# Grice-Lab/HmmUFOtu

Hardware: AMD Instinct MI355X
Metric: reads placed/sec (whole node), gg_97_otus GTR+dGamma 250bp; HBM GB/s %peak (higher is better)
Workload: dtype f64; 1 GPU; gg_97_otus-scale synthetic DB (198643 nodes x 7682 CS columns, K=1400), GTR+dGamma(4), SE 250 bp amplicon reads, batch 8192 reads/step/GPU, 6 batches in flight, seeds in the reference's std::sort order (k_seed_refsort); seed_order=reference, message_window_cols=7682, parallelism=read-sharded x1

## Files before the change

hmmufotu_amd/csrc/hu_common.h:

```cpp
#pragma once
#include <hip/hip_runtime.h>
#include <stdint.h>
#include <string>
#include <functional>
#include <istream>
#include <ostream>
#include <vector>
#include <exception>
#include <mutex>
#include <thread>
#include "../../include/hmmufotu_amd.h"

#define HU_MAX_DGK 16
#define HU_READ_TILE 16
#define HU_MAX_INS 24
#define HU_TILEQ_MASK_SHIFT 16
#define HU_TILEW_QUAD (4 * HU_READ_TILE * 3)
#define HU_NODE_PAD 256
#define HU_MIN_LOGLIK_EXP (-510.0)
#define HU_BRANCH_EPS 1e-5
#define HU_MAX_ITER 100

struct HuModelDev {
	int32_t type, dgK;
	double pi[4];
	double logpi[4];
	double U[16], U1[16], lam[4];
	double rate[HU_MAX_DGK];
};

struct HuDbDev {
	int32_t nNodes, nNodesPad, csLen, W, WQ, root;
	int64_t winStart, winLen;
	const uint4* planes;
	const int32_t* posCol;
	const unsigned long long* colPlanes;
	int32_t QM, pad0;
	const uint2* nodeCover;
	const int32_t* parent;
	const double* blen;
	const double* height;
	const double* up;
	const double* down;
	const int32_t* upK;
	const int32_t* downK;
	int32_t K, L;
	const double* EM;
	const double* EI;
	const double* T;
	const double* entryC;
	const double* exitC;
	const int32_t* p2cs;
	const double* Tt;
	const double* EMt;
	const double* EIt;
	const double* placeConst;
	int32_t rLo, rHi;
	const uint32_t* wideList;
};
__device__ inline bool hu_skip_width(const HuDbDev& db, int cols) { return db.rHi != 0 && (cols <= db.rLo || cols > db.rHi); }

struct HuRegion {
	int32_t j0, j1, i0, i1;
	int32_t withB;
	int32_t band;
	int32_t from, start, nIns, nDel;
	int64_t off;
	int64_t doff;
	int32_t ci0, cj0;
	int64_t coff;
};
#define HU_MAX_REGIONS 6
#define HU_READ_NEEDS_VALUES 8

struct HuReadDesc {
	int64_t baseOff;
	int32_t len;
	int32_t nRegions;
	int64_t scratchOff;
	int64_t traceOff;
	int64_t decOff;
	int64_t cornerOff;
	HuRegion reg[HU_MAX_REGIONS];
};

void hu_set_error(const char* fmt, ...);
int hu_catch_all(const char* fn) noexcept;
void hu_sort_prefix_packed(uint64_t* a, size_t n, size_t k);

#define HU_PC_LAM 0
#define HU_PC_RATE 4
#define HU_PC_W 20
#define HU_PC_C 100
#define HU_PC_CB 164
#define HU_PC_S 184
#define HU_PC_COUNT 188
void hu_place_consts(const HuModelDev& m, double* pc);

int hu_model_prepare(const hu_model_desc* d, HuModelDev* out);

// ... 49 lines not shown
```

hmmufotu_amd/csrc/hu_engine.hip:

```cpp
#include <algorithm>
#include <cmath>
#include <cstdio>
#include <cstring>
#include <limits>
#include <map>
#include <atomic>
#include <thread>
#include <memory>
#include <mutex>
#include <chrono>
#include <fstream>
#include <sstream>
#include <new>
#include <stdexcept>
#include <fcntl.h>
#include <unistd.h>
#include "hu_common.h"
#include "hu_kern_sep.h"
#include "hu_kern_align.h"
#include "hu_kern_tree.h"
#include "hu_kern_blk.h"
#include "hu_kern_refsort.h"
#include "hu_kern_rank.h"
#include "hu_kern_anneal.h"
// ... 1841 lines not shown
			if(g2.i1 >= g2.i0 && g2.j1 >= g2.j0) { nearI = std::min(nearI, g2.i0 - 1); nearJ = std::min(nearJ, g2.j0 - 1); }
		}
		g.ci0 = std::max(g.i0, nearI); g.cj0 = std::max(g.j0, nearJ); g.coff = coff;
		if(nearI == INT32_MAX || g.ci0 > g.i1 || g.cj0 > g.j1 || g.i1 < g.i0 || g.j1 < g.j0) { g.ci0 = g.i1 + 1; g.cj0 = g.j1 + 1; }
		else coff += (int64_t)(g.i1 - g.ci0 + 1) * (g.j1 - g.cj0 + 1);
	}
	rd.scratchOff = off;
	rd.decOff = doff;
	rd.cornerOff = coff;
}

static int upload_descs(hu_batch* b) {
	int rc;
	if((rc = b->dDescs.ensure(b->hDescs.size())) != HU_OK) return rc;
	HIPCHK(hipMemcpyAsync(b->dDescs.p, b->hDescs.data(), b->hDescs.size() * sizeof(HuReadDesc), hipMemcpyHostToDevice, b->stream));
	return HU_OK;
}

extern "C" int hu_batch_set_reads(hu_batch* b, int n, const char* bases, const int64_t* offs, const int32_t* vpaths,
		const char* mates, const int64_t* moffs, const int32_t* mvpaths) try {
	if(!b || n < 0 || n > b->maxReads || (n > 0 && (!bases || !offs))) { hu_set_error("hu_batch_set_reads: bad argument"); return HU_ERR_ARG; }
	if(mates && !moffs) { hu_set_error("hu_batch_set_reads: mates without offsets"); return HU_ERR_ARG; }
	HIPCHK(hipSetDevice(b->db->device));
	b->n = n; b->paired = mates != nullptr; b->nSeq = b->paired ? 2 * n : n; b->fromCodes = false;
	b->hDescs.assign(b->nSeq, HuReadDesc());
	b->hBases.clear();
	b->maxBases = 0;
	for(int r = 0; r < n; ++r) {
		const int64_t l = (offs[r + 1] - offs[r]) + (mates ? moffs[r + 1] - moffs[r] : 0);
		if(l > b->maxBases) b->maxBases = (int) std::min<int64_t>(l, 1 << 30);
	}
	int64_t cells = 0, tr = 0, decs = 0, corners = 0;
	for(int s = 0; s < b->nSeq; ++s) {
		const bool isMate = s >= n;
		const int r = isMate ? s - n : s;
		const char* src = isMate ? mates + moffs[r] : bases + offs[r];
		const int64_t len64 = isMate ? moffs[r + 1] - moffs[r] : offs[r + 1] - offs[r];
		HuReadDesc& rd = b->hDescs[s];
		memset(&rd, 0, sizeof(rd));
		rd.baseOff = (int64_t) b->hBases.size();
		rd.len = (int32_t) len64;
		bool bad = len64 < 1 || len64 > 65535;
		for(int64_t i = 0; i < len64 && !bad; ++i) if(host_sym(src[i]) < 0) bad = true;
		if(!bad) {
			b->hBases.insert(b->hBases.end(), src, src + len64);
			const int32_t* vp = isMate ? (mvpaths ? mvpaths + (size_t) r * 12 : nullptr) : (vpaths ? vpaths + (size_t) r * 12 : nullptr);
			build_regions(b->db, rd.len, vp, rd);
			const int64_t c = rd.scratchOff, dc = rd.decOff, cc = rd.cornerOff;
			rd.scratchOff = cells; cells += c;
			rd.decOff = decs; decs += dc;
			rd.cornerOff = corners; corners += cc;
		}
		else { rd.len = 0; rd.nRegions = 0; }
		rd.traceOff = tr;
		tr += rd.len + b->db->dev.K + 8;
	}
	int rc;
	if((rc = b->dBases.ensure(b->hBases.size() + 1)) != HU_OK) return rc;
	b->cellsTotal = cells; b->cornerTotal = corners;
	if((rc = b->dDec.ensure((size_t) decs + 1)) != HU_OK) return rc;
	if((rc = b->dTraces.ensure((size_t) tr + 1)) != HU_OK) return rc;
	if((rc = b->dVit.ensure(b->nSeq)) != HU_OK) return rc;
	if(!b->hBases.empty()) HIPCHK(hipMemcpyAsync(b->dBases.p, b->hBases.data(), b->hBases.size(), hipMemcpyHostToDevice, b->stream));
	if((rc = upload_descs(b)) != HU_OK) return rc;
	b->state = ST_READS;
	return HU_OK;
} catch(...) { return hu_catch_all("hu_batch_set_reads"); }

static int ensure_read_buffers(hu_batch* b) {
	const HuDbDev& d = b->db->dev;
	const size_t n = (size_t) b->n;
	const size_t tiles = (n + HU_READ_TILE - 1) / HU_READ_TILE;
	int rc;
	if((rc = b->dCodes.ensure(n * d.csLen)) != HU_OK) return rc;
	if((rc = b->dStart.ensure(n)) != HU_OK) return rc;
	if((rc = b->dEnd.ensure(n)) != HU_OK) return rc;
	if((rc = b->dRp.ensure(tiles * d.WQ * HU_READ_TILE * 16)) != HU_OK) return rc;
	if((rc = b->dTileQ.ensure(tiles * (d.WQ + 1))) != HU_OK) return rc;
	if((rc = b->dTileW.ensure(std::max<size_t>(tiles, 1) * d.WQ * HU_TILEW_QUAD)) != HU_OK) return rc;
	if((rc = b->dSlotRead.ensure(std::max<size_t>(tiles, 1) * HU_READ_TILE)) != HU_OK) return rc;
	if((rc = b->dReadSlot.ensure(std::max<size_t>(n, 1))) != HU_OK) return rc;
	if((rc = b->dRq.ensure(std::max<size_t>(n, 1) * ((d.WQ + 31) / 32))) != HU_OK) return rc;
	if((rc = b->dIns.ensure(std::max<size_t>(n, 1) * (HU_MAX_INS + 1))) != HU_OK) return rc;
	if((rc = b->dTileIns.ensure(std::max<size_t>(tiles, 1) * (HU_READ_TILE * HU_MAX_INS + 1))) != HU_OK) return rc;
	if((rc = b->dRSpan.ensure(std::max<size_t>(n, 1) * 2)) != HU_OK) return rc;
	if((rc = b->dTileSpan.ensure(std::max<size_t>(tiles, 1) * 2)) != HU_OK) return rc;
	return HU_OK;
}

static int order_by_key(hu_batch* b, const uint32_t* key, const uint32_t* val, size_t n, uint32_t bound, uint32_t* out, bool runsInOrder) {
	if(!n) return HU_OK;
	const size_t m = (size_t) bound + 1;
	int rc;
	const size_t nTiles = (m + 1023) / 1024;
	if((rc = b->dCsCnt.ensure(3 * m + nTiles + 8)) != HU_OK) return rc;
	uint32_t* cnt = b->dCsCnt.p; uint32_t* start = cnt + m; uint32_t* cur = start + m + 1; uint32_t* tiles = cur + m;
	HIPCHK(hipMemsetAsync(cnt, 0, m * 4, b->stream));
	k_cs_hist<<<(unsigned)((n + 255) / 256), 256, 0, b->stream>>>((int) n, key, bound, cnt);
	k_cs_tile_sums<<<(unsigned) nTiles, 1024, 0, b->stream>>>((int) m, cnt, tiles);
	k_cs_scan_tiles<<<1, 1024, 0, b->stream>>>((int) nTiles, tiles);
	k_cs_scan<<<(unsigned) nTiles, 1024, 0, b->stream>>>((int) m, cnt, tiles, start, cur);
	k_cs_scatter<<<(unsigned)((n + 255) / 256), 256, 0, b->stream>>>((int) n, key, val, bound, cur, out);
	if(runsInOrder) k_cs_runs<<<(unsigned)((m + 3) / 4), 256, 0, b->stream>>>((int) bound, start, out);
	HIPCHK(hipGetLastError());
	return HU_OK;
}

static int tile_reads(hu_batch* b, const HuAlnDev* alns) {
	const int n = b->n;
	if(!n) return HU_OK;
	const int tiles = (n + HU_READ_TILE - 1) / HU_READ_TILE;
	int rc;
	if((rc = b->dSortK.ensure((size_t) n * 2)) != HU_OK || (rc = b->dSortV.ensure((size_t) n * 2)) != HU_OK) return rc;
	k_tile_keys<<<(n + 255) / 256, 256, 0, b->stream>>>(n, alns, b->dStart.p, b->dEnd.p, b->dSortK.p, b->dSortV.p);
	if(b->knob.tile_unsorted) HIPCHK(hipMemcpyAsync(b->dSortV.p + n, b->dSortV.p, (size_t) n * 4, hipMemcpyDeviceToDevice, b->stream));
	else if((rc = order_by_key(b, b->dSortK.p, b->dSortV.p, (size_t) n, (uint32_t) b->db->dev.csLen + 1u, b->dSortV.p + n, true)) != HU_OK) return rc;
	k_tile_slots<<<(tiles * HU_READ_TILE + 255) / 256, 256, 0, b->stream>>>(n, tiles * HU_READ_TILE, b->dSortV.p + n, b->dSlotRead.p, b->dReadSlot.p);
	HIPCHK(hipGetLastError());
	return HU_OK;
}

static int set_aligned_impl(hu_batch* b, int n, const int8_t* codes, hipMemcpyKind kind, const int32_t* start, const int32_t* end, int maxBases = -1) {
	if(!b || n < 0 || n > b->maxReads || (n > 0 && (!codes || !start || !end))) { hu_set_error("hu_batch_set_aligned: bad argument"); return HU_ERR_ARG; }
	HIPCHK(hipSetDevice(b->db->device));
	const HuDbDev& d = b->db->dev;
	b->n = n; b->nSeq = n; b->paired = false; b->fromCodes = true;
	if(maxBases >= 0) b->maxBases = maxBases;
	else {
		int mb = 0;
		for(int r = 0; r < n; ++r) {
			if(!(start[r] >= 0 && start[r] <= end[r] && end[r] < d.csLen)) continue;
			const int8_t* c = codes + (size_t) r * d.csLen; int k = 0;
			for(int j = start[r]; j <= end[r]; ++j) k += c[j] >= 0;
			mb = std::max(mb, k);
		}
		b->maxBases = mb;
	}
	int rc;
	if((rc = ensure_read_buffers(b)) != HU_OK) return rc;
	b->hAlns.assign(n, HuAlnDev());
	b->hStart.assign(start, start + n); b->hEnd.assign(end, end + n);
	for(int r = 0; r < n; ++r) {
		HuAlnDev& a = b->hAlns[r];
		memset(&a, 0, sizeof(a));
		const bool ok = start[r] >= 0 && start[r] <= end[r] && end[r] < d.csLen && start[r] >= d.winStart && end[r] < d.winStart + d.winLen;
		a.status = ok ? HU_READ_OK : HU_READ_INVALID;
		a.csStart = start[r] + 1; a.csEnd = end[r] + 1;
		if(!ok) { b->hStart[r] = (int32_t) d.winStart; b->hEnd[r] = (int32_t) d.winStart - 1; }
	}
	(void) hipGetLastError();
	if(n) {
		if((const void*) codes != (const void*) b->dCodes.p) HIPCHK(hipMemcpyAsync(b->dCodes.p, codes, (size_t) n * d.csLen, kind, b->stream));
		HIPCHK(hipMemcpyAsync(b->dStart.p, b->hStart.data(), (size_t) n * 4, hipMemcpyHostToDevice, b->stream));
		HIPCHK(hipMemcpyAsync(b->dEnd.p, b->hEnd.data(), (size_t) n * 4, hipMemcpyHostToDevice, b->stream));
		const int tiles = (n + HU_READ_TILE - 1) / HU_READ_TILE;
		HIPCHK(hipMemsetAsync(b->dRp.p, 0, (size_t) tiles * d.WQ * HU_READ_TILE * 16 * 4, b->stream));
		if((rc = tile_reads(b, nullptr)) != HU_OK) return rc;
		k_planes_from_codes<<<n, 64, 0, b->stream>>>(d, b->dCodes.p, b->dStart.p, b->dEnd.p, b->dRp.p, b->dRq.p, b->dIns.p, b->dReadSlot.p, (uint2*) b->dRSpan.p);
		k_tile_lists<<<tiles, 64, 0, b->stream>>>(d, n, b->dRp.p, b->dRq.p, b->dIns.p, b->dTileQ.p, b->dTileW.p, b->dTileIns.p, b->dSlotRead.p, (const uint2*) b->dRSpan.p, (uint2*) b->dTileSpan.p);
		HIPCHK(hipGetLastError());
	}
	b->state = ST_ALIGNED;
	return HU_OK;
}
extern "C" int hu_batch_set_aligned(hu_batch* b, int n, const int8_t* codes, const int32_t* start, const int32_t* end) try {
	return set_aligned_impl(b, n, codes, hipMemcpyHostToDevice, start, end);
} catch(...) { return hu_catch_all("hu_batch_set_aligned"); }
// ... 1975 lines not shown
```

hmmufotu_amd/csrc/hu_kern_align.h:

```cpp
#pragma once
#include "hu_common.h"

struct HuVitOut { int32_t alnStart, alnEnd, alnFrom, alnTo, traceLen, status; double minScore; };

__device__ inline bool reg_contains(const HuRegion& g, int i, int j) {
	if(j < g.j0 || j > g.j1 || i < g.i0 || i > g.i1) return false;
	if(g.band) { int dist = (i - g.from) - (j - g.start); if(!(dist <= g.nIns && dist >= -g.nDel)) return false; }
	return true;
}

struct VitCtx {
	const HuReadDesc* rd;
	const double* scr;
	double tNN, tNB;
};

__device__ inline void vit_lookup(const VitCtx& c, int upto, int i, int j, double& m, double& ii, double& d) {
	const HuReadDesc& rd = *c.rd;
	for(int r = upto - 1; r >= 0; --r) {
		const HuRegion& g = rd.reg[r];
		if(reg_contains(g, i, j)) {
			const int64_t idx = (g.off + (int64_t)(j - g.j0) * (g.i1 - g.i0 + 1) + (i - g.i0)) * 3;
			m = c.scr[idx]; ii = c.scr[idx + 1]; d = c.scr[idx + 2];
			return;
// ... 1060 lines not shown
	}
	if(lane == 0) {
		if(db.WQ & 31) qbits[(db.WQ - 1) >> 5] = acc; il[0] = li;
		rspan[r] = make_uint2((any1 ? f1 : 0xffffu) | ((any1 ? l1 : 0u) << 16), (any2 ? f2 : 0xffffu) | ((any2 ? l2 : 0u) << 16));
	}
}

__global__ __launch_bounds__(64) void k_encode_rows(HuDbDev db, const char* __restrict__ rows, HuAlnDev* __restrict__ alns,
		int8_t* __restrict__ codes, int32_t* __restrict__ rstart, int32_t* __restrict__ rend, uint32_t* __restrict__ rp, uint32_t* __restrict__ rq,
		int32_t* __restrict__ ins, const int32_t* __restrict__ readSlot, uint2* __restrict__ rspan) {
	const int r = blockIdx.x, lane = threadIdx.x;
	const HuAlnDev a = alns[r];
	const char* row = rows + (size_t) r * db.csLen;
	int8_t* cd = codes + (size_t) r * db.csLen;
	bool ok = a.status == HU_READ_OK;
	if(ok && (a.csStart - 1 < db.winStart || a.csEnd - 1 >= db.winStart + db.winLen)) {
		ok = false;
		if(lane == 0) alns[r].status = HU_READ_OUT_OF_WINDOW;
	}
	const int start = ok ? a.csStart - 1 : (int) db.winStart, end = ok ? a.csEnd - 1 : (int) db.winStart - 1;
	if(lane == 0) { rstart[r] = start; rend[r] = end; }
	for(int c = lane; c < db.csLen; c += 64) {
		char ch = row[c];
		if(ch >= 'a' && ch <= 'z') ch = (char)(ch - 32);
		cd[c] = c_sym_map[(int) ch & 127];
	}
	__syncthreads();
	planes_of_codes(db, cd, start, end, r, readSlot[r], lane, rp, rq, ins, rspan);
}

__global__ __launch_bounds__(64) void k_planes_from_codes(HuDbDev db, const int8_t* __restrict__ codes,
		const int32_t* __restrict__ rstart, const int32_t* __restrict__ rend, uint32_t* __restrict__ rp, uint32_t* __restrict__ rq,
		int32_t* __restrict__ ins, const int32_t* __restrict__ readSlot, uint2* __restrict__ rspan) {
	const int r = blockIdx.x, lane = threadIdx.x;
	planes_of_codes(db, codes + (size_t) r * db.csLen, rstart[r], rend[r], r, readSlot[r], lane, rp, rq, ins, rspan);
}

__global__ void k_tile_keys(int n, const HuAlnDev* __restrict__ alns, const int32_t* __restrict__ rstart, const int32_t* __restrict__ rend,
		uint32_t* __restrict__ key, uint32_t* __restrict__ val) {
	const int r = blockIdx.x * 256 + threadIdx.x;
	if(r >= n) return;
	uint32_t k;
	if(alns) k = alns[r].status == HU_READ_OK ? (uint32_t) alns[r].csStart : 0x7fffffffu;
	else k = rend[r] >= rstart[r] ? (uint32_t) rstart[r] + 1u : 0x7fffffffu;
	key[r] = k; val[r] = (uint32_t) r;
}
__global__ void k_tile_slots(int n, int nSlots, const uint32_t* __restrict__ sortedRead, int32_t* __restrict__ slotRead, int32_t* __restrict__ readSlot) {
	const int s = blockIdx.x * 256 + threadIdx.x;
	if(s >= nSlots) return;
	if(s < n) { const int r = (int) sortedRead[s]; slotRead[s] = r; readSlot[r] = s; }
	else slotRead[s] = -1;
}

__global__ __launch_bounds__(64) void k_tile_lists(HuDbDev db, int n, const uint32_t* __restrict__ rp, const uint32_t* __restrict__ rq, const int32_t* __restrict__ ins,
		int32_t* __restrict__ tileQ, uint32_t* __restrict__ tileW, int32_t* __restrict__ tileIns, const int32_t* __restrict__ slotRead, const uint2* __restrict__ rspan,
		uint2* __restrict__ tileSpan) {
	static_assert(HU_READ_TILE == 16, "sixteen reads x four validity words of a quad = one dword per lane");
	const int tile = blockIdx.x, lane = threadIdx.x;
	const int nw32 = (db.WQ + 31) / 32;
	int32_t* out = tileQ + (size_t) tile * (db.WQ + 1);
	uint32_t* wout = tileW + (size_t) tile * db.WQ * HU_TILEW_QUAD;
	int cnt = 0;
	for(int w = 0; w < nw32; ++w) {
		uint32_t m = 0;
		if(lane < HU_READ_TILE) { const int r = slotRead[tile * HU_READ_TILE + lane]; if(r >= 0) m = rq[(size_t) r * nw32 + w]; }
		for(int s = 32; s > 0; s >>= 1) m |= __shfl_xor(m, s);
		while(m) {
			const int q = w * 32 + __ffs(m) - 1; m &= m - 1;
			const uint32_t* __restrict__ rt = rp + ((size_t) tile * db.WQ + q) * (HU_READ_TILE * 16);
			unsigned long long b = __ballot(rt[(lane >> 2) * 16 + 8 + (lane & 3)] != 0u);
			b |= b >> 32; b |= b >> 16; b |= b >> 8; b |= b >> 4;
			uint32_t mk = (uint32_t) b & 15u;
			if(lane == 0) out[1 + cnt] = q | (int) mk << HU_TILEQ_MASK_SHIFT;
			++cnt;
			while(mk) {
				const int wd = __ffs(mk) - 1; mk &= mk - 1;
				if(lane < HU_READ_TILE * 3) wout[lane] = rt[(lane / 3) * 16 + (lane % 3) * 4 + wd];
				wout += HU_READ_TILE * 3;
			}
		}
	}
	if(lane == 0) {
		out[0] = cnt;
		int32_t* til = tileIns + (size_t) tile * (HU_READ_TILE * HU_MAX_INS + 1);
		int ne = 0;
		for(int t = 0; t < HU_READ_TILE; ++t) {
			const int r = slotRead[tile * HU_READ_TILE + t];
			if(r < 0) continue;
			const int32_t* il = ins + (size_t) r * (HU_MAX_INS + 1);
			for(int e = 0; e < il[0]; ++e) til[1 + ne++] = (t << 24) | il[1 + e];
		}
		til[0] = ne;
		uint32_t f1 = 0xffffu, l1 = 0, f2 = 0xffffu, l2 = 0; bool a1 = false, a2 = false;
		for(int t = 0; t < HU_READ_TILE; ++t) {
			const int r = slotRead[tile * HU_READ_TILE + t];
			if(r < 0) continue;
			const uint2 s2 = rspan[r];
			if((s2.x & 0xffffu) <= (s2.x >> 16)) { f1 = a1 ? min(f1, s2.x & 0xffffu) : (s2.x & 0xffffu); l1 = a1 ? max(l1, s2.x >> 16) : (s2.x >> 16); a1 = true; }
			if((s2.y & 0xffffu) <= (s2.y >> 16)) { f2 = a2 ? min(f2, s2.y & 0xffffu) : (s2.y & 0xffffu); l2 = a2 ? max(l2, s2.y >> 16) : (s2.y >> 16); a2 = true; }
		}
		tileSpan[tile] = make_uint2((a1 ? f1 : 0xffffu) | ((a1 ? l1 : 0u) << 16), (a2 ? f2 : 0xffffu) | ((a2 ? l2 : 0u) << 16));
	}
}
```

hmmufotu_amd/csrc/hu_kern_sep.h:

```cpp
#pragma once
#include "hu_common.h"

#define HU_TOPK_BINS 4097
#define HU_TOPK_CAP 4096

template<class PT> struct HuPair;
template<> struct HuPair<uint32_t> {
	static constexpr int PPV = 4;
	__device__ static inline uint32_t canon(uint32_t x) { return x; }
	__device__ static inline uint32_t pack(uint32_t c) { return c; }
	__device__ static inline void unpack(const uint4& v, uint32_t* o) { o[0] = v.x; o[1] = v.y; o[2] = v.z; o[3] = v.w; }
};
template<> struct HuPair<uint16_t> {
	static constexpr int PPV = 8;
	__device__ static inline uint32_t canon(uint32_t x) { return ((x >> 8) << 16) | (x & 0xffu); }
	__device__ static inline uint16_t pack(uint32_t c) { return (uint16_t)(((c >> 16) << 8) | (c & 0xffu)); }
	__device__ static inline void unpack(const uint4& v, uint32_t* o) {
		const uint32_t w[4] = {v.x, v.y, v.z, v.w};
#pragma unroll
		for(int e = 0; e < 8; ++e) o[e] = canon((w[e >> 1] >> ((e & 1) * 16)) & 0xffffu);
	}
};
__device__ inline uint32_t hu_pair_load(const void* pairs, size_t idx, int p16) {
	return p16 ? HuPair<uint16_t>::canon(((const uint16_t*) pairs)[idx]) : ((const uint32_t*) pairs)[idx];
}

__global__ __launch_bounds__(64) void k_col_planes(HuDbDev db, unsigned long long* __restrict__ col) {
	const int nb = blockIdx.x, q = db.QM + blockIdx.y, lane = threadIdx.x;
	const size_t np = (size_t) db.nNodesPad, npw = np / 64;
	const int node = nb * 64 + lane;
	for(int p = 0; p < 3; ++p) {
		const uint4 v = db.planes[((size_t) q * 3 + p) * np + node];
		const uint32_t w[4] = {v.x, v.y, v.z, v.w};
		for(int i = 0; i < 128; ++i) {
			const unsigned long long m = __ballot((w[i >> 5] >> (i & 31)) & 1u);
			if(lane == 0) col[(((size_t) blockIdx.y * 128 + i) * 3 + p) * npw + nb] = m;
		}
	}
}

__global__ __launch_bounds__(256) void k_node_cover(HuDbDev db, uint2* __restrict__ cover) {
	const int node = blockIdx.x * 256 + threadIdx.x;
	if(node >= db.nNodesPad) return;
	uint32_t f1 = 0xffffu, l1 = 0, f2 = 0xffffu, l2 = 0; bool any1 = false, any2 = false;
	for(int q = 0; q < db.WQ; ++q) {
		const uint4 v = db.planes[((size_t) q * 3 + 2) * db.nNodesPad + node];
		const uint32_t w[4] = {v.x, v.y, v.z, v.w};
		for(int k = 0; k < 4; ++k) {
			if(!w[k]) continue;
			const uint32_t lo = (uint32_t) q * 128 + k * 32 + (__ffs(w[k]) - 1), hi = (uint32_t) q * 128 + k * 32 + 31 - __clz(w[k]);
			if(q < db.QM) { if(!any1) { f1 = lo; any1 = true; } l1 = hi; }
			else { if(!any2) { f2 = lo; any2 = true; } l2 = hi; }
		}
	}
	cover[node] = make_uint2((any1 ? f1 : 0xffffu) | ((any1 ? l1 : 0u) << 16), (any2 ? f2 : 0xffffu) | ((any2 ? l2 : 0u) << 16));
}
__device__ inline bool hu_span_meets(uint32_t a, uint32_t b) {
	return (a & 0xffffu) <= (b >> 16) && (b & 0xffffu) <= (a >> 16) && (a & 0xffffu) <= (a >> 16) && (b & 0xffffu) <= (b >> 16);
}
__device__ inline bool hu_cover_meets(uint2 node, uint2 read) { return hu_span_meets(node.x, read.x) || hu_span_meets(node.y, read.y); }

template<int CTRL>
__device__ inline uint32_t dpp_min_full(uint32_t v) {
	const uint32_t o = (uint32_t) __builtin_amdgcn_mov_dpp((int) v, CTRL, 0xf, 0xf, true);
	return o < v ? o : v;
}
__device__ __forceinline__ void hu_scan_word(uint32_t n0, uint32_t n1, uint32_t nv, const uint32_t* __restrict__ r, uint32_t (&d)[HU_READ_TILE], uint32_t (&N)[HU_READ_TILE]) {
#pragma unroll
	for(int t = 0; t < HU_READ_TILE; ++t) {
		const uint32_t k = nv & r[t * 3 + 2], x = ((n0 ^ r[t * 3]) | (n1 ^ r[t * 3 + 1])) & k;
		d[t] += __popc(x); N[t] += __popc(k);
	}
}

template<class PT, bool L0 = false>
__global__ __launch_bounds__(256, 8) void k_seed_pdist2(HuDbDev db, const uint32_t* __restrict__ tileW,
		const int32_t* __restrict__ tileQ, const int32_t* __restrict__ tileIns, PT* __restrict__ pairs, const int32_t* __restrict__ slotRead,
		uint32_t* __restrict__ piv = nullptr, unsigned long long* __restrict__ l0m = nullptr) {
	constexpr int T = HU_READ_TILE;
	__shared__ uint32_t acc[T][256];
	const int tile = blockIdx.x, tid = threadIdx.x;
	const int node = blockIdx.y * 256 + tid;
	const int32_t* __restrict__ ql = tileQ + (size_t) tile * (db.WQ + 1);
	const int32_t* __restrict__ til = tileIns + (size_t) tile * (T * HU_MAX_INS + 1);
	const int nq = ql[0], ne = til[0];
	uint32_t d[T], N[T];
#pragma unroll
	for(int t = 0; t < T; ++t) { d[t] = 0; N[t] = 0; }
	if(ne) {
#pragma unroll
		for(int t = 0; t < T; ++t) acc[t][tid] = 0;
	}
	const size_t np = (size_t) db.nNodesPad;
	const uint32_t* __restrict__ wr = (const uint32_t*) __builtin_assume_aligned(tileW + (size_t) tile * db.WQ * HU_TILEW_QUAD, 64);
	for(int qi = 0; qi < nq; ++qi) {
		const int ent = ql[1 + qi], q = ent & ((1 << HU_TILEQ_MASK_SHIFT) - 1);
		const uint4 n0 = db.planes[((size_t) q * 3 + 0) * np + node], n1 = db.planes[((size_t) q * 3 + 1) * np + node], nv = db.planes[((size_t) q * 3 + 2) * np + node];
		if(ent & (1 << HU_TILEQ_MASK_SHIFT)) { hu_scan_word(n0.x, n1.x, nv.x, wr, d, N); wr += T * 3; }
		if(ent & (2 << HU_TILEQ_MASK_SHIFT)) { hu_scan_word(n0.y, n1.y, nv.y, wr, d, N); wr += T * 3; }
		if(ent & (4 << HU_TILEQ_MASK_SHIFT)) { hu_scan_word(n0.z, n1.z, nv.z, wr, d, N); wr += T * 3; }
		if(ent & (8 << HU_TILEQ_MASK_SHIFT)) { hu_scan_word(n0.w, n1.w, nv.w, wr, d, N); wr += T * 3; }
	}
	{
		const size_t npw = np / 64;
		const int nb = __builtin_amdgcn_readfirstlane(node >> 6), lane = tid & 63;
		for(int e = 0; e < ne; ++e) {
			const int ent = til[1 + e];
			const int t = ent >> 24, pos = (ent >> 2) & 0x3fffff, code = ent & 3;
			const unsigned long long* cp = db.colPlanes + ((size_t)(pos - db.QM * 128) * 3) * npw + nb;
			const unsigned long long W0 = cp[0], W1 = cp[npw], Wv = cp[2 * npw];
			const uint32_t valid = (uint32_t)(Wv >> lane) & 1u, nc = ((uint32_t)(W0 >> lane) & 1u) | (((uint32_t)(W1 >> lane) & 1u) << 1);
			const uint32_t add = valid | ((valid & (nc != (uint32_t) code ? 1u : 0u)) << 16);
			atomicAdd(&acc[t][tid], add);
		}
	}
	const bool counts = L0 && node < db.nNodes && node != db.root;
	bool zero = false;
#pragma unroll
	for(int t = 0; t < T; ++t) {
		const int read = slotRead[tile * T + t];
		if(read >= 0) {
			const uint32_t v = ((d[t] << 16) | N[t]) + (ne ? acc[t][tid] : 0u);
			pairs[(size_t) read * np + node] = HuPair<PT>::pack(v);
			if(L0) {
				const uint32_t pp = piv[(size_t) read * 4];
				const uint32_t a = (v >> 16) * (pp & 0xffffu), bb = (pp >> 16) * (v & 0xffffu);
				const unsigned long long mL = __ballot(counts && a >= bb), mR = __ballot(counts && bb >= a);
				if((tid & 63) == 0) *reinterpret_cast<ulonglong2*>(l0m + ((size_t) read * (np / 64) + (size_t)(node >> 6)) * 2) = make_ulonglong2(mL, mR);
				zero |= v == 0u;
			}
		}
	}
	if(L0 && __ballot(zero && counts)) {
#pragma unroll
		for(int t = 0; t < T; ++t) {
			const int read = slotRead[tile * T + t];
			if(read < 0) continue;
			const uint32_t v = ((d[t] << 16) | N[t]) + (ne ? acc[t][tid] : 0u);
			if(__ballot(counts && v == 0u) && (tid & 63) == 0) atomicOr(&piv[(size_t) read * 4 + 3], 1u);
		}
	}
}

template<class DT>
__global__ __launch_bounds__(256, 3) void k_seed_dscan4(HuDbDev db, const uint32_t* __restrict__ rp,
		const int32_t* __restrict__ tileQ, DT* __restrict__ dm, const int32_t* __restrict__ slotRead, uint32_t* __restrict__ bminD, const uint2* __restrict__ tileSpan) {
	constexpr int T = HU_READ_TILE, M = 4;
	constexpr uint32_t DMAX = (uint32_t)(DT) ~(DT) 0;
	static_assert(T == 16, "sixteen reads x sixteen dwords per quad = one dword per thread");
	__shared__ __attribute__((aligned(16))) uint32_t rpl2[2][T * 16];
	__shared__ __attribute__((aligned(16))) uint32_t mb[4][T][64];
	const int tile = blockIdx.x, tid = threadIdx.x, lane = tid & 63, wave = tid >> 6;
	const int node0 = blockIdx.y * (256 * M) + tid * M;
	const bool live = node0 < db.nNodesPad;
	const int nl = live ? node0 : 0;
	const int32_t* __restrict__ ql = tileQ + (size_t) tile * (db.WQ + 1);
	const int nq = ql[0];
	uint32_t d[T][M];
#pragma unroll
	for(int t = 0; t < T; ++t)
#pragma unroll
		for(int m = 0; m < M; ++m) d[t][m] = 0;
	const size_t np = (size_t) db.nNodesPad;
	for(int qi = 0; qi < nq; ++qi) {
		const int q = ql[1 + qi] & ((1 << HU_TILEQ_MASK_SHIFT) - 1);
		const uint32_t mine = rp[((size_t) tile * db.WQ + q) * (T * 16) + tid];
		uint4 n0[M], n1[M], nv[M];
#pragma unroll
		for(int m = 0; m < M; ++m) {
			n0[m] = db.planes[((size_t) q * 3 + 0) * np + nl + m]; n1[m] = db.planes[((size_t) q * 3 + 1) * np + nl + m]; nv[m] = db.planes[((size_t) q * 3 + 2) * np + nl + m];
		}
		uint32_t* rpl = rpl2[qi & 1];
		rpl[tid] = mine;
		__syncthreads();
		uint4 r0 = *reinterpret_cast<const uint4*>(&rpl[0]), r1 = *reinterpret_cast<const uint4*>(&rpl[4]), rv = *reinterpret_cast<const uint4*>(&rpl[8]);
#pragma unroll
		for(int t = 0; t < T; ++t) {
			const int tn = t + 1 < T ? t + 1 : t;
			const uint4 p0 = *reinterpret_cast<const uint4*>(&rpl[tn * 16]), p1 = *reinterpret_cast<const uint4*>(&rpl[tn * 16 + 4]), pv = *reinterpret_cast<const uint4*>(&rpl[tn * 16 + 8]);
			uint32_t a[M][4];
#pragma unroll
			for(int m = 0; m < M; ++m) { a[m][0] = n0[m].x ^ r0.x; a[m][1] = n0[m].y ^ r0.y; a[m][2] = n0[m].z ^ r0.z; a[m][3] = n0[m].w ^ r0.w; }
			__builtin_amdgcn_sched_barrier(0);
#pragma unroll
			for(int m = 0; m < M; ++m) {
				a[m][0] = __builtin_amdgcn_bitop3_b32(a[m][0], n1[m].x, r1.x, 0xf6); a[m][1] = __builtin_amdgcn_bitop3_b32(a[m][1], n1[m].y, r1.y, 0xf6);
				a[m][2] = __builtin_amdgcn_bitop3_b32(a[m][2], n1[m].z, r1.z, 0xf6); a[m][3] = __builtin_amdgcn_bitop3_b32(a[m][3], n1[m].w, r1.w, 0xf6);
			}
			__builtin_amdgcn_sched_barrier(0);
#pragma unroll
			for(int m = 0; m < M; ++m) {
				a[m][0] = __builtin_amdgcn_bitop3_b32(a[m][0], nv[m].x, rv.x, 0x80); a[m][1] = __builtin_amdgcn_bitop3_b32(a[m][1], nv[m].y, rv.y, 0x80);
				a[m][2] = __builtin_amdgcn_bitop3_b32(a[m][2], nv[m].z, rv.z, 0x80); a[m][3] = __builtin_amdgcn_bitop3_b32(a[m][3], nv[m].w, rv.w, 0x80);
			}
			__builtin_amdgcn_sched_barrier(0);
#pragma unroll
			for(int w = 0; w < 4; ++w) {
#pragma unroll
				for(int m = 0; m < M; ++m) asm("v_bcnt_u32_b32 %0, %1, %0" : "+v"(d[t][m]) : "v"(a[m][w]));
			}
			__builtin_amdgcn_sched_barrier(0);
			r0 = p0; r1 = p1; rv = pv;
		}
	}
	uint32_t skip[M];
	const uint2 tsp = tileSpan[tile];
#pragma unroll
	for(int m = 0; m < M; ++m) skip[m] = live && node0 + m < db.nNodes && node0 + m != db.root && hu_cover_meets(db.nodeCover[nl + m], tsp) ? 0u : 0xffffffffu;
#pragma unroll
	for(int t = 0; t < T; ++t) {
		const int read = slotRead[tile * T + t];
		uint32_t v[M];
#pragma unroll
		for(int m = 0; m < M; ++m) v[m] = min(d[t][m], DMAX);
		if(read >= 0 && live) {
			DT* dst = dm + (size_t) read * np + node0;
			if(sizeof(DT) == 1) *reinterpret_cast<uint32_t*>(dst) = v[0] | (v[1] << 8) | (v[2] << 16) | (v[3] << 24);
			else *reinterpret_cast<uint2*>(dst) = make_uint2(v[0] | (v[1] << 16), v[2] | (v[3] << 16));
		}
		mb[wave][t][lane] = min(min(v[0] | skip[0], v[1] | skip[1]), min(v[2] | skip[2], v[3] | skip[3]));
	}
	__syncthreads();
// ... 1224 lines not shown
```

Measured before the change: 416,000 reads/s.

## Replace LDS atomics in seed pdist kernel with wave-uniform register accumulation

```diff
diff --git a/hmmufotu_amd/csrc/hu_common.h b/hmmufotu_amd/csrc/hu_common.h
--- a/hmmufotu_amd/csrc/hu_common.h
+++ b/hmmufotu_amd/csrc/hu_common.h
@@ -16,6 +16,7 @@
 #define HU_MAX_INS 24
 #define HU_TILEQ_MASK_SHIFT 16
 #define HU_TILEW_QUAD (4 * HU_READ_TILE * 3)
+#define HU_TILEINS_STRIDE (HU_READ_TILE * (HU_MAX_INS + 1))
 #define HU_NODE_PAD 256
 #define HU_MIN_LOGLIK_EXP (-510.0)
 #define HU_BRANCH_EPS 1e-5
diff --git a/hmmufotu_amd/csrc/hu_engine.hip b/hmmufotu_amd/csrc/hu_engine.hip
--- a/hmmufotu_amd/csrc/hu_engine.hip
+++ b/hmmufotu_amd/csrc/hu_engine.hip
@@ -1947,7 +1947,7 @@
 	if((rc = b->dReadSlot.ensure(std::max<size_t>(n, 1))) != HU_OK) return rc;
 	if((rc = b->dRq.ensure(std::max<size_t>(n, 1) * ((d.WQ + 31) / 32))) != HU_OK) return rc;
 	if((rc = b->dIns.ensure(std::max<size_t>(n, 1) * (HU_MAX_INS + 1))) != HU_OK) return rc;
-	if((rc = b->dTileIns.ensure(std::max<size_t>(tiles, 1) * (HU_READ_TILE * HU_MAX_INS + 1))) != HU_OK) return rc;
+	if((rc = b->dTileIns.ensure(std::max<size_t>(tiles, 1) * HU_TILEINS_STRIDE)) != HU_OK) return rc;
 	if((rc = b->dRSpan.ensure(std::max<size_t>(n, 1) * 2)) != HU_OK) return rc;
 	if((rc = b->dTileSpan.ensure(std::max<size_t>(tiles, 1) * 2)) != HU_OK) return rc;
 	return HU_OK;
diff --git a/hmmufotu_amd/csrc/hu_kern_align.h b/hmmufotu_amd/csrc/hu_kern_align.h
--- a/hmmufotu_amd/csrc/hu_kern_align.h
+++ b/hmmufotu_amd/csrc/hu_kern_align.h
@@ -1166,15 +1166,16 @@
 	}
 	if(lane == 0) {
 		out[0] = cnt;
-		int32_t* til = tileIns + (size_t) tile * (HU_READ_TILE * HU_MAX_INS + 1);
+		int32_t* til = tileIns + (size_t) tile * HU_TILEINS_STRIDE;
 		int ne = 0;
 		for(int t = 0; t < HU_READ_TILE; ++t) {
 			const int r = slotRead[tile * HU_READ_TILE + t];
-			if(r < 0) continue;
-			const int32_t* il = ins + (size_t) r * (HU_MAX_INS + 1);
-			for(int e = 0; e < il[0]; ++e) til[1 + ne++] = (t << 24) | il[1 + e];
-		}
-		til[0] = ne;
+			if(r >= 0) {
+				const int32_t* il = ins + (size_t) r * (HU_MAX_INS + 1);
+				for(int e = 0; e < il[0]; ++e) til[HU_READ_TILE + ne++] = (t << 24) | il[1 + e];
+			}
+			til[t] = ne;
+		}
 		uint32_t f1 = 0xffffu, l1 = 0, f2 = 0xffffu, l2 = 0; bool a1 = false, a2 = false;
 		for(int t = 0; t < HU_READ_TILE; ++t) {
 			const int r = slotRead[tile * HU_READ_TILE + t];
diff --git a/hmmufotu_amd/csrc/hu_kern_sep.h b/hmmufotu_amd/csrc/hu_kern_sep.h
--- a/hmmufotu_amd/csrc/hu_kern_sep.h
+++ b/hmmufotu_amd/csrc/hu_kern_sep.h
@@ -1,5 +1,6 @@
 #pragma once
 #include "hu_common.h"
+#include <utility>
 
 #define HU_TOPK_BINS 4097
 #define HU_TOPK_CAP 4096
@@ -9,12 +10,14 @@
 	static constexpr int PPV = 4;
 	__device__ static inline uint32_t canon(uint32_t x) { return x; }
 	__device__ static inline uint32_t pack(uint32_t c) { return c; }
+	__device__ static inline uint32_t pack2(uint32_t d, uint32_t N) { return (d << 16) | N; }
 	__device__ static inline void unpack(const uint4& v, uint32_t* o) { o[0] = v.x; o[1] = v.y; o[2] = v.z; o[3] = v.w; }
 };
 template<> struct HuPair<uint16_t> {
 	static constexpr int PPV = 8;
 	__device__ static inline uint32_t canon(uint32_t x) { return ((x >> 8) << 16) | (x & 0xffu); }
 	__device__ static inline uint16_t pack(uint32_t c) { return (uint16_t)(((c >> 16) << 8) | (c & 0xffu)); }
+	__device__ static inline uint16_t pack2(uint32_t d, uint32_t N) { return (uint16_t)((d << 8) | N); }
 	__device__ static inline void unpack(const uint4& v, uint32_t* o) {
 		const uint32_t w[4] = {v.x, v.y, v.z, v.w};
 #pragma unroll
@@ -73,24 +76,31 @@
 	}
 }
 
+template<int LANE>
+__device__ __forceinline__ void hu_writelane(uint32_t& v, uint32_t s) { asm("v_writelane_b32 %0, %1, %2" : "+v"(v) : "s"(s), "n"(LANE)); }
+template<class F, int... I>
+__device__ __forceinline__ void hu_static_for(F&& f, std::integer_sequence<int, I...>) { (f(std::integral_constant<int, I>{}), ...); }
+
 template<class PT, bool L0 = false>
 __global__ __launch_bounds__(256, 8) void k_seed_pdist2(HuDbDev db, const uint32_t* __restrict__ tileW,
 		const int32_t* __restrict__ tileQ, const int32_t* __restrict__ tileIns, PT* __restrict__ pairs, const int32_t* __restrict__ slotRead,
 		uint32_t* __restrict__ piv = nullptr, unsigned long long* __restrict__ l0m = nullptr) {
 	constexpr int T = HU_READ_TILE;
-	__shared__ uint32_t acc[T][256];
-	const int tile = blockIdx.x, tid = threadIdx.x;
+	static_assert(T <= 64, "slot t's read, pivot and masks live in lane t");
+	const int tile = blockIdx.x, tid = threadIdx.x, lane = tid & 63;
 	const int node = blockIdx.y * 256 + tid;
 	const int32_t* __restrict__ ql = tileQ + (size_t) tile * (db.WQ + 1);
-	const int32_t* __restrict__ til = tileIns + (size_t) tile * (T * HU_MAX_INS + 1);
-	const int nq = ql[0], ne = til[0];
+	const int32_t* __restrict__ til = tileIns + (size_t) tile * HU_TILEINS_STRIDE;
+	const int nq = ql[0];
+	int vread = -1, vend = 0; uint32_t vpiv = 0;
+	int vent = til[T + lane];
+	if(lane < T) {
+		vread = slotRead[tile * T + lane]; vend = til[lane];
+		if(L0 && vread >= 0) vpiv = piv[(size_t) vread * 4];
+	}
 	uint32_t d[T], N[T];
 #pragma unroll
 	for(int t = 0; t < T; ++t) { d[t] = 0; N[t] = 0; }
-	if(ne) {
-#pragma unroll
-		for(int t = 0; t < T; ++t) acc[t][tid] = 0;
-	}
 	const size_t np = (size_t) db.nNodesPad;
 	const uint32_t* __restrict__ wr = (const uint32_t*) __builtin_assume_aligned(tileW + (size_t) tile * db.WQ * HU_TILEW_QUAD, 64);
 	for(int qi = 0; qi < nq; ++qi) {
@@ -101,43 +111,55 @@
 		if(ent & (4 << HU_TILEQ_MASK_SHIFT)) { hu_scan_word(n0.z, n1.z, nv.z, wr, d, N); wr += T * 3; }
 		if(ent & (8 << HU_TILEQ_MASK_SHIFT)) { hu_scan_word(n0.w, n1.w, nv.w, wr, d, N); wr += T * 3; }
 	}
-	{
+	if(__builtin_amdgcn_readlane(vend, T - 1)) {
 		const size_t npw = np / 64;
-		const int nb = __builtin_amdgcn_readfirstlane(node >> 6), lane = tid & 63;
-		for(int e = 0; e < ne; ++e) {
-			const int ent = til[1 + e];
-			const int t = ent >> 24, pos = (ent >> 2) & 0x3fffff, code = ent & 3;
-			const unsigned long long* cp = db.colPlanes + ((size_t)(pos - db.QM * 128) * 3) * npw + nb;
-			const unsigned long long W0 = cp[0], W1 = cp[npw], Wv = cp[2 * npw];
-			const uint32_t valid = (uint32_t)(Wv >> lane) & 1u, nc = ((uint32_t)(W0 >> lane) & 1u) | (((uint32_t)(W1 >> lane) & 1u) << 1);
-			const uint32_t add = valid | ((valid & (nc != (uint32_t) code ? 1u : 0u)) << 16);
-			atomicAdd(&acc[t][tid], add);
+		const uint32_t npw3 = (uint32_t)(3 * npw);
+		const int nb = __builtin_amdgcn_readfirstlane(node >> 6);
+		int e = 0, base = 0;
+#pragma unroll
+		for(int t = 0; t < T; ++t) {
+			const int end = __builtin_amdgcn_readlane(vend, t);
+			for(; e < end; ++e) {
+				if(e >= base + 64) { base += 64; vent = til[T + base + lane]; }
+				const int ent = __builtin_amdgcn_readlane(vent, e - base);
+				const uint32_t pos = ((uint32_t) ent >> 2) & 0x3fffffu;
+				const unsigned long long* cp = db.colPlanes + (unsigned long long)(pos - (uint32_t)(db.QM * 128)) * npw3 + nb;
+				const unsigned long long W0 = cp[0], W1 = cp[npw], Wv = cp[2 * npw];
+				const unsigned long long c0 = (ent & 1) ? ~0ull : 0ull, c1 = (ent & 2) ? ~0ull : 0ull;
+				const unsigned long long mm = Wv & ((W0 ^ c0) | (W1 ^ c1));
+				N[t] += __builtin_amdgcn_inverse_ballot_w64(Wv) ? 1u : 0u;
+				d[t] += __builtin_amdgcn_inverse_ballot_w64(mm) ? 1u : 0u;
+			}
 		}
 	}
 	const bool counts = L0 && node < db.nNodes && node != db.root;
-	bool zero = false;
-#pragma unroll
-	for(int t = 0; t < T; ++t) {
-		const int read = slotRead[tile * T + t];
+	const unsigned long long cm = L0 ? __ballot(counts) : 0ull;
+	uint32_t mk0 = 0, mk1 = 0, mk2 = 0, mk3 = 0;
+	unsigned long long zm = 0;
+	hu_static_for([&](auto tc) {
+		constexpr int t = decltype(tc)::value;
+		const int read = __builtin_amdgcn_readlane(vread, t);
+		const uint32_t pp = (uint32_t) __builtin_amdgcn_readlane((int) vpiv, t);
 		if(read >= 0) {
-			const uint32_t v = ((d[t] << 16) | N[t]) + (ne ? acc[t][tid] : 0u);
-			pairs[(size_t) read * np + node] = HuPair<PT>::pack(v);
+			pairs[(size_t) read * np + node] = HuPair<PT>::pack2(d[t], N[t]);
 			if(L0) {
-				const uint32_t pp = piv[(size_t) read * 4];
-				const uint32_t a = (v >> 16) * (pp & 0xffffu), bb = (pp >> 16) * (v & 0xffffu);
-				const unsigned long long mL = __ballot(counts && a >= bb), mR = __ballot(counts && bb >= a);
-				if((tid & 63) == 0) *reinterpret_cast<ulonglong2*>(l0m + ((size_t) read * (np / 64) + (size_t)(node >> 6)) * 2) = make_ulonglong2(mL, mR);
-				zero |= v == 0u;
-			}
-		}
-	}
-	if(L0 && __ballot(zero && counts)) {
-#pragma unroll
-		for(int t = 0; t < T; ++t) {
-			const int read = slotRead[tile * T + t];
-			if(read < 0) continue;
-			const uint32_t v = ((d[t] << 16) | N[t]) + (ne ? acc[t][tid] : 0u);
-			if(__ballot(counts && v == 0u) && (tid & 63) == 0) atomicOr(&piv[(size_t) read * 4 + 3], 1u);
+				const uint32_t a = __umul24(d[t], pp & 0xffffu), bb = __umul24(pp >> 16, N[t]);
+				const unsigned long long mL = __ballot(a >= bb) & cm, mR = __ballot(bb >= a) & cm;
+				hu_writelane<t>(mk0, (uint32_t) mL); hu_writelane<t>(mk1, (uint32_t)(mL >> 32));
+				hu_writelane<t>(mk2, (uint32_t) mR); hu_writelane<t>(mk3, (uint32_t)(mR >> 32));
+				zm |= __ballot(N[t] == 0u);
+			}
+		}
+	}, std::make_integer_sequence<int, T>{});
+	if(L0) {
+		if(vread >= 0) *reinterpret_cast<uint4*>(l0m + ((size_t) vread * (np / 64) + (size_t)(node >> 6)) * 2) = make_uint4(mk0, mk1, mk2, mk3);
+		if(zm & cm) {
+#pragma unroll
+			for(int t = 0; t < T; ++t) {
+				const int read = __builtin_amdgcn_readlane(vread, t);
+				if(read < 0) continue;
+				if((__ballot(N[t] == 0u) & cm) && lane == 0) atomicOr(&piv[(size_t) read * 4 + 3], 1u);
+			}
 		}
 	}
 }
```

New measurement: 424,600 reads/s (median of 6 runs). 1.02x the previous value.
